# tumberger/gnark-fork

Hardware: AMD Instinct MI355X
Metric: Groth16 prove time + MSM G1 throughput (Mscalar-mul/s) BN254 2^24 R1CS, 1/2/4/8 GPU (higher is better)
Workload: dtype u32 limbs (BN254 Fp/Fr Montgomery, integer)

## Files before the change

### gnark-fork_amd/csrc/groth16.hip

```cpp
#include "common.h"
#include "curve.cuh"
#include "stage.h"
#include <chrono>
#include <future>
#include <memory>
#include <mutex>
#include <thread>
#include <vector>
#include <cstdlib>
#include <cstring>

struct gg_domain;
struct gg_msm_base;

namespace gg {
struct MsmSort;
struct MsmScratch;
struct MsmWork;
void compute_h_device(gg_domain* d, Fr* A, Fr* B, Fr* C, Fr* H, hipStream_t st);
void msm_device(gg_msm_base* b, const Fr* scalars_dev, void* out_jac, hipStream_t st);
size_t msm_scalars_needed(gg_msm_base* b);
gg_msm_base* msm_base_create_internal(int group, const void* host_points, size_t n,
                                      const uint32_t* sidx, int window_bits, bool keep_inf, int groups);
int choose_groups_multi(const double* bytes, const int* W, int k, double extra);
bool msm_same_shape(const gg_msm_base* a, const gg_msm_base* b);
MsmSort* msm_own_sort(gg_msm_base* b);
void msm_prepare_dev(gg_msm_base* b, MsmSort* s, const Fr* scalars_dev, hipStream_t st, int slog = 0,
                     uint32_t sres = 0);
void msm_finish_dev(gg_msm_base* b, MsmSort* s, void* out_jac, hipStream_t st, MsmScratch* scr = nullptr);
MsmWork* msm_work_new();
void msm_work_delete(MsmWork* w);
MsmSort* msm_work_sort(MsmWork* w);
void msm_prepare_derived_dev(gg_msm_base* a, MsmSort* sa, gg_msm_base* b, MsmSort* sb, const uint32_t* bmap,
                             hipStream_t st);
bool msm_derivable(const gg_msm_base* a, const gg_msm_base* b);
void msm_build_bmap(const gg_msm_base* a, const gg_msm_base* b, DevBuf& bmap);
MsmScratch* msm_work_scratch(MsmWork* w);
int msm_base_window(const gg_msm_base* b);
int choose_c(size_t n, size_t point_bytes, int total_bits);
void hshard_run(gg_hshard* hs, const Fr* a, const Fr* b, const Fr* c, size_t len, bool compact, Fr* send,
                Fr* recv, gg_exchange_fn xchg, void* ctx, hipStream_t st);
size_t hshard_m(const gg_hshard* hs, int* rank, int* world, int* log_n);
Fr* hshard_h(gg_hshard* hs);
int hshard_curve(const gg_hshard* hs);
}

struct DistH {
    gg_hshard* hs;
    gg_exchange_fn xchg;
    void* ctx;
    gg::Fr *send, *recv;
};

using namespace gg;

struct CurveBn254 {
    using FrT = Fr;
    using G1F = Fp;
    using G2F = Fp2;
    static constexpr int curve = GG_CURVE_BN254, g1 = GG_G1, g2 = GG_G2, total_bits = 255;
};
struct CurveBls12381 {
    using FrT = FrBls;
    using G1F = FpBls;
    using G2F = Fp2Bls;
    static constexpr int curve = GG_CURVE_BLS12_381, g1 = GG_BLS12_381_G1, g2 = GG_BLS12_381_G2, total_bits = 256;
};
struct PointSizes {
    size_t g1a, g2a, g1j, g2j;
};
static PointSizes point_sizes(int curve) {
    if (curve == GG_CURVE_BN254) return {64, 128, 96, 192};
// ... 5 lines not shown
    bool share_AK = false, share_B = false;
    bool derive_B = false;
    DevBuf bmap;
    int groups = 1;
    WireBases() = default;
    WireBases(const WireBases&) = delete;
    WireBases& operator=(const WireBases&) = delete;
    ~WireBases() {
        for (gg_msm_base_t b : {A, B, K, B2})
            if (b) gg_msm_base_release(b);
    }
};

struct WorkSet {
    MsmWork *A = nullptr, *B = nullptr, *K = nullptr, *B2 = nullptr;
    WorkSet() {
        A = msm_work_new();
        B = msm_work_new();
        K = msm_work_new();
        B2 = msm_work_new();
    }
    WorkSet(const WorkSet&) = delete;
    WorkSet& operator=(const WorkSet&) = delete;
    ~WorkSet() {
        for (MsmWork* w : {A, B, K, B2})
            if (w) msm_work_delete(w);
    }
};

struct gg_groth16_pk {
    int curve = GG_CURVE_BN254;
    int log_n = 0;
    size_t n = 0;
    gg_domain_t dom = nullptr;
    std::shared_ptr<WireBases> wb;
    gg_msm_base_t A = nullptr, B = nullptr, K = nullptr, Z = nullptr, B2 = nullptr;
    int slog = 0;
    uint32_t spart = 0;
    std::unique_ptr<WorkSet> work;
    uint8_t alpha[96], beta[96], delta[96], beta2[192], delta2[192];
    size_t n_wires = 0, nb_public = 0;
    size_t wire_lo = 0, wire_hi = 0, z_lo = 0, nZ = 0;
    bool share_AK = false, share_B = false;
    DevBuf wires, sa, sb, sc;
    hipStream_t s0 = nullptr, s1 = nullptr, s2 = nullptr, s3 = nullptr, s4 = nullptr;
    TaskQueue tq[5];
    hipStream_t* const* active() {
        act[0] = &s0, act[1] = &s1, act[2] = &s2, act[3] = &s3, act[4] = &s4;
        return act;
    }
    hipStream_t* act[5] = {};
    hipStream_t hprio = nullptr;
    std::unique_ptr<Stager> stager;
    int device = 0;
    std::mutex mu;
    ~gg_groth16_pk() {
        stager.reset();
        work.reset();
        wb.reset();
        if (Z) gg_msm_base_release(Z);
        if (dom) gg_domain_release(dom);
        task_streams_release(tq, 5, device);
        if (hprio) (void)hipStreamDestroy(hprio);
    }
};

static thread_local double g_timings[9];
static thread_local double g_ext[3];

static void ck(int rc) {
    if (rc != GG_OK) throw Error(rc, gg_last_error());
}

static std::shared_ptr<WireBases> wire_bases_build(int curve, int log_n, const void* g1_A, size_t nA,
                                                   const void* g1_B, size_t nB, const void* g1_K, size_t nK,
                                                   const void* g2_B, const uint8_t* inf_A, const uint8_t* inf_B,
                                                   size_t n_wires, size_t nb_public, const uint32_t* k_wire_index,
                                                   size_t lo, size_t hi, size_t nZ) {
    GG_CHECK(inf_A && inf_B, GG_ERR_INVALID_ARG, "null infinity masks");
    GG_CHECK(nb_public <= n_wires, GG_ERR_INVALID_ARG, "nb_public > n_wires");
    GG_CHECK(lo <= hi && hi <= n_wires, GG_ERR_INVALID_ARG, "bad wire shard range");
    GG_CHECK(curve == GG_CURVE_BN254 || curve == GG_CURVE_BLS12_381, GG_ERR_INVALID_ARG, "bad curve");
    const PointSizes ps = point_sizes(curve);
    const int g1 = curve == GG_CURVE_BN254 ? GG_G1 : GG_BLS12_381_G1;
    const int g2 = curve == GG_CURVE_BN254 ? GG_G2 : GG_BLS12_381_G2;
    const int tbits = curve == GG_CURVE_BN254 ? 255 : 256;
    std::vector<uint32_t> ia, ib, ik;
    for (size_t i = lo; i < hi; i++) {
        if (!inf_A[i]) ia.push_back((uint32_t)(i - lo));
        if (!inf_B[i]) ib.push_back((uint32_t)(i - lo));
    }
    GG_CHECK(ia.size() == nA, GG_ERR_INVALID_ARG, "len(pk.G1.A) != n_wires - NbInfinityA (shard)");
    GG_CHECK(ib.size() == nB, GG_ERR_INVALID_ARG, "len(pk.G1.B) != n_wires - NbInfinityB (shard)");
    ik.resize(nK);
    const size_t k0 = std::max(lo, nb_public);
    for (size_t i = 0; i < nK; i++) {
        size_t w = k_wire_index ? (size_t)k_wire_index[i] : k0 + i;
        GG_CHECK(w >= lo && w < hi, GG_ERR_INVALID_ARG, "K wire index outside the shard");
        ik[i] = (uint32_t)(w - lo);
    }
    GG_CHECK(nA == 0 || g1_A, GG_ERR_INVALID_ARG, "null g1_A");
    GG_CHECK(nB == 0 || (g1_B && g2_B), GG_ERR_INVALID_ARG, "null g1_B / g2_B");
    GG_CHECK(nK == 0 || g1_K, GG_ERR_INVALID_ARG, "null g1_K");
    const size_t nw = hi - lo;
    const int cAK = choose_c(std::max<size_t>(nw, 1), ps.g1a, tbits);
    int cB = choose_c(std::max<size_t>(nB, 1), 128, tbits);
    const bool try_derive = getenv("GG_G16_B_DERIVE") && atoi(getenv("GG_G16_B_DERIVE")) != 0;
    if (try_derive && cAK >= cB && cAK - cB <= 2 && nB) cB = cAK;
    if (const char* e = getenv("GG_G16_B_WINDOW")) cB = std::max(4, std::min(24, atoi(e)));
// ... 39 lines not shown
                      const void* omega_mont, const void* coset_gen_mont, const void* g1_Z, size_t z_lo, size_t nZ,
                      const void* alpha1, const void* beta1, const void* delta1, const void* beta2,
                      const void* delta2, size_t n_wires, size_t nb_public, size_t lo, size_t hi, int slog,
                      uint32_t spart) {
    GG_CHECK(omega_mont && coset_gen_mont && alpha1 && beta1 && delta1 && beta2 && delta2,
             GG_ERR_INVALID_ARG, "null argument");
    GG_CHECK(log_n >= 0 && log_n <= 28, GG_ERR_INVALID_ARG, "log_n out of range");
    const PointSizes ps = point_sizes(curve);
    const int g1 = curve == GG_CURVE_BN254 ? GG_G1 : GG_BLS12_381_G1;
    const int tbits = curve == GG_CURVE_BN254 ? 255 : 256;
    pk->curve = curve;
    pk->log_n = log_n;
    pk->n = (size_t)1 << log_n;
    pk->n_wires = n_wires;
    pk->nb_public = nb_public;
    pk->wire_lo = lo;
    pk->wire_hi = hi;
    pk->z_lo = z_lo;
    pk->nZ = nZ;
    const size_t nz_full = pk->n > 1 ? pk->n - 1 : 0;
    GG_CHECK(z_lo + nZ <= nz_full, GG_ERR_INVALID_ARG,
             "Z shard beyond domain cardinality - 1 (setup.go:266)");
    GG_CHECK(nZ == 0 || g1_Z, GG_ERR_INVALID_ARG, "null g1_Z");
    GG_HIP(hipGetDevice(&pk->device));
    memcpy(pk->alpha, alpha1, ps.g1a);
    memcpy(pk->beta, beta1, ps.g1a);
    memcpy(pk->delta, delta1, ps.g1a);
    memcpy(pk->beta2, beta2, ps.g2a);
    memcpy(pk->delta2, delta2, ps.g2a);
    ck(gg_domain_create_ex(curve, log_n, omega_mont, coset_gen_mont, &pk->dom));
    pk->wb = std::move(wb);
    pk->A = pk->wb->A;
    pk->B = pk->wb->B;
    pk->K = pk->wb->K;
    pk->B2 = pk->wb->B2;
    pk->share_AK = pk->wb->share_AK;
    pk->share_B = pk->wb->share_B;
    if (slog) {
        int cmin = 64;
        for (gg_msm_base_t b : {pk->A, pk->B})
            if (msm_scalars_needed(b)) cmin = std::min(cmin, msm_base_window(b));
        GG_CHECK(slog <= cmin - 2, GG_ERR_INVALID_ARG, "bucket stripe too fine for the tables' windows");
        GG_CHECK(spart < (1u << slog), GG_ERR_INVALID_ARG, "stripe part out of range");
        pk->slog = slog;
        pk->spart = spart;
        pk->work.reset(new WorkSet());
    }
    const int cZ = choose_c(std::max<size_t>(nZ, 1), ps.g1a, tbits);
    pk->Z = msm_base_create_internal(g1, g1_Z, nZ, nullptr, cZ, false, pk->wb->groups);
    int cur = 0;
    GG_HIP(hipGetDevice(&cur));
    task_streams_init(pk->active(), pk->tq, 5, cur, true);
    h_priority_ab(pk);
}

static void pk_build(gg_groth16_pk* pk, int curve, int log_n, const void* omega_mont, const void* coset_gen_mont,
                     const void* g1_A, size_t nA, const void* g1_B, size_t nB, const void* g1_Z,
                     size_t z_lo, size_t nZ, const void* g1_K, size_t nK, const void* alpha1,
                     const void* beta1, const void* delta1, const void* g2_B, const void* beta2,
                     const void* delta2, const uint8_t* inf_A, const uint8_t* inf_B, size_t n_wires,
                     size_t nb_public, const uint32_t* k_wire_index, size_t lo, size_t hi) {
    GG_CHECK(log_n >= 0 && log_n <= 28, GG_ERR_INVALID_ARG, "log_n out of range");
    auto wb = wire_bases_build(curve, log_n, g1_A, nA, g1_B, nB, g1_K, nK, g2_B, inf_A, inf_B, n_wires, nb_public,
                               k_wire_index, lo, hi, nZ);
    pk_finish(pk, std::move(wb), curve, log_n, omega_mont, coset_gen_mont, g1_Z, z_lo, nZ, alpha1, beta1, delta1,
              beta2, delta2, n_wires, nb_public, lo, hi, 0, 0);
}

namespace gg {
std::shared_ptr<WireBases> g16_wire_bases(int curve, int log_n, const void* g1_A, size_t nA, const void* g1_B,
                                          size_t nB, const void* g1_K, size_t nK, const void* g2_B,
                                          const uint8_t* inf_A, const uint8_t* inf_B, size_t n_wires,
                                          size_t nb_public, const uint32_t* k_wire_index, size_t nZ) {
    return wire_bases_build(curve, log_n, g1_A, nA, g1_B, nB, g1_K, nK, g2_B, inf_A, inf_B, n_wires, nb_public,
                            k_wire_index, 0, n_wires, nZ);
}
gg_groth16_pk* g16_stripe_shard(std::shared_ptr<WireBases> wb, int curve, int log_n, const void* omega_mont,
                                const void* coset_gen_mont, const void* g1_Z, size_t z_lo, size_t nZ,
                                const void* alpha1, const void* beta1, const void* delta1, const void* beta2,
                                const void* delta2, size_t n_wires, size_t nb_public, int slog, uint32_t spart) {
    std::unique_ptr<gg_groth16_pk> pk(new gg_groth16_pk());
    pk_finish(pk.get(), std::move(wb), curve, log_n, omega_mont, coset_gen_mont, g1_Z, z_lo, nZ, alpha1, beta1,
              delta1, beta2, delta2, n_wires, nb_public, 0, n_wires, slog, spart);
    return pk.release();
}
int g16_wire_window(int curve, size_t n_wires, size_t nB) {
    const PointSizes ps = point_sizes(curve);
    const int tbits = curve == GG_CURVE_BN254 ? 255 : 256;
    int c = 64;
    if (n_wires) c = std::min(c, choose_c(n_wires, ps.g1a, tbits));
    if (nB) c = std::min(c, choose_c(nB, 128, tbits));
    return c;
}
void g16_restream(gg_groth16_pk* pk, bool dedicated) {
    std::lock_guard<std::mutex> lk(pk->mu);
    task_streams_switch(pk->active(), pk->tq, 5, pk->device, dedicated);
    h_priority_ab(pk);
}
}

extern "C" int gg_groth16_pk_create_ex(int curve, int log_n, const void* omega_mont, const void* coset_gen_mont,
                                       const void* g1_A, size_t nA, const void* g1_B, size_t nB,
                                       const void* g1_Z, size_t nZ, const void* g1_K, size_t nK,
                                       const void* alpha1, const void* beta1, const void* delta1,
                                       const void* g2_B, const void* beta2, const void* delta2,
                                       const uint8_t* inf_A, const uint8_t* inf_B, size_t n_wires,
// ... 120 lines not shown
        .count();
}

template <class T>
static T from_bytes(const void* p) {
    T x;
    memcpy(&x, p, sizeof(T));
    return x;
}

struct G16Partials {
    alignas(16) uint8_t a[144], b1[144], k[144], z[144];
    alignas(16) uint8_t b2[288];
};
static void set_g1_inf(int curve, void* p) {
    if (curve == GG_CURVE_BN254) {
        G1Jac j = G1Jac::inf();
        memcpy(p, &j, sizeof(j));
    } else {
        Jac<FpBls> j = Jac<FpBls>::inf();
        memcpy(p, &j, sizeof(j));
    }
}
static void partials_put(int curve, const G16Partials& p, void* out) {
    const PointSizes ps = point_sizes(curve);
    uint8_t* o = (uint8_t*)out;
    memcpy(o, p.a, ps.g1j);
    memcpy(o + ps.g1j, p.b1, ps.g1j);
    memcpy(o + 2 * ps.g1j, p.k, ps.g1j);
    memcpy(o + 3 * ps.g1j, p.z, ps.g1j);
    memcpy(o + 4 * ps.g1j, p.b2, ps.g2j);
}
static void partials_get(int curve, const void* in, G16Partials& p) {
    const PointSizes ps = point_sizes(curve);
    const uint8_t* q = (const uint8_t*)in;
    memcpy(p.a, q, ps.g1j);
    memcpy(p.b1, q + ps.g1j, ps.g1j);
    memcpy(p.k, q + 2 * ps.g1j, ps.g1j);
    memcpy(p.z, q + 3 * ps.g1j, ps.g1j);
    memcpy(p.b2, q + 4 * ps.g1j, ps.g2j);
}

struct Joiner {
    std::vector<gg::Task<void>>& v;
    ~Joiner() {
        for (auto& t : v)
            if (t.valid()) t.wait();
    }
};

static void prove_device(gg_groth16_pk* pk, const void* wires, const void* sol_a,
                         const void* sol_b, const void* sol_c, size_t n_cons,
                         bool inputs_on_device, void* h_dev_out, G16Partials& out,
                         const DistH* dh = nullptr) {
    double t0 = now_ms();
    const size_t n = pk->n;
    const size_t nbytes = n * 32;
    const size_t nw_shard = pk->wire_hi - pk->wire_lo;
    const Fr* wdev = (const Fr*)wires;
    if (!inputs_on_device) {
        if (!pk->stager) pk->stager.reset(new Stager(pk->device));
        pk->wires.reserve(std::max<size_t>(nw_shard, 1) * 32);
        pk->stager->upload(pk->wires.p, (const uint8_t*)wires + pk->wire_lo * 32, nw_shard * 32);
        const hipStream_t cons[4] = {pk->s0, pk->s2, pk->s3, pk->s4};
        pk->stager->ready(cons, 4);
        wdev = pk->wires.as<Fr>();
    } else {
        wdev += pk->wire_lo;
    }
    double t_up = now_ms();

    set_g1_inf(pk->curve, out.z);
    double t_h = 0, t_z = 0, t_a = 0, t_b = 0, t_k = 0, t_upabc = 0;
    std::mutex emu;
    std::string werr;
    int wcode = GG_OK;
    const int dev = pk->device;
    auto guarded = [&](auto fn) {
        return [&, fn]() {
            try {
                GG_HIP(hipSetDevice(dev));
                fn();
            } catch (const Error& e) {
                std::lock_guard<std::mutex> g(emu);
                if (wcode == GG_OK) { werr = e.what(); wcode = e.code; }
            } catch (const std::exception& e) {
                std::lock_guard<std::mutex> g(emu);
                if (wcode == GG_OK) { werr = e.what(); wcode = GG_ERR_INTERNAL; }
            }
        };
    };
    const bool serial = getenv("GG_G16_SERIAL") && atoi(getenv("GG_G16_SERIAL"));
    std::vector<gg::Task<void>> workers;
    Joiner joiner{workers};
    auto spawn = [&](auto fn) {
        if (serial) fn();
        else workers.push_back(gg::run_task(fn));
    };
    auto inputs_abc = [&](Fr*& A, Fr*& B, Fr*& C, size_t& len) {
        const void* src[3] = {sol_a, sol_b, sol_c};
        Fr* dst[3] = {pk->sa.as<Fr>(), pk->sb.as<Fr>(), pk->sc.as<Fr>()};
        len = n_cons;
        const double a = now_ms();
        if (inputs_on_device) {
            for (int i = 0; i < 3; i++) {
                if (dh) { dst[i] = (Fr*)src[i]; continue; }
                if (n_cons) GG_HIP(hipMemcpyAsync(dst[i], src[i], n_cons * 32, hipMemcpyDeviceToDevice, pk->s1));
                if (n_cons < n) GG_HIP(hipMemsetAsync((char*)dst[i] + n_cons * 32, 0, nbytes - n_cons * 32, pk->s1));
            }
        } else if (dh) {
            int rank = 0, world = 1, lg = 0;
            hshard_m(dh->hs, &rank, &world, &lg);
            len = n_cons > (size_t)rank ? (n_cons - (size_t)rank + world - 1) / world : 0;
            for (int i = 0; i < 3; i++)
                pk->stager->upload_strided(dst[i], src[i], 32, (size_t)rank, (size_t)world, len);
            pk->stager->ready(&pk->s1, 1);
        } else {
            for (int i = 0; i < 3; i++) {
                if (n_cons < n) GG_HIP(hipMemsetAsync((char*)dst[i] + n_cons * 32, 0, nbytes - n_cons * 32, pk->s1));
                pk->stager->upload(dst[i], src[i], n_cons * 32);
            }
            pk->stager->ready(&pk->s1, 1);
        }
        t_upabc = now_ms() - a;
        A = dst[0];
        B = dst[1];
        C = dst[2];
    };
    pk->sa.reserve(nbytes);
    pk->sb.reserve(nbytes);
    pk->sc.reserve(nbytes);
    if (dh) spawn(guarded([&] {
        Fr *A, *B, *C;
        size_t len;
        double a = now_ms();
        inputs_abc(A, B, C, len);
        const bool compact = !inputs_on_device;
        hshard_run(dh->hs, A, B, C, len, compact, dh->send, dh->recv, dh->xchg, dh->ctx, pk->s1);
        GG_WAIT_STREAM(pk->s1);
        double b = now_ms();
        t_h = b - a;
        msm_device(pk->Z, hshard_h(dh->hs), out.z, pk->s1);
        t_z = now_ms() - b;
    }));
    else spawn(guarded([&] {
        Fr *A, *B, *C;
        size_t len;
        double a = now_ms();
        inputs_abc(A, B, C, len);
        compute_h_device(pk->dom, A, B, C, A, pk->s1);
        GG_WAIT_STREAM(pk->s1);
        double b = now_ms();
        t_h = b - a;
        if (h_dev_out) GG_HIP(hipMemcpyAsync(h_dev_out, A, nbytes, hipMemcpyDeviceToDevice, pk->s1));
        if (n > 1) msm_device(pk->Z, A + pk->z_lo, out.z, pk->s1);
        t_z = now_ms() - b;
    }));
    MsmSort *sAK = nullptr, *sB = nullptr, *sK = nullptr, *sB2 = nullptr;
    MsmScratch *xA = nullptr, *xB = nullptr, *xK = nullptr, *xB2 = nullptr;
    WorkSet* ws = pk->work.get();
    guarded([&] {
        sAK = ws ? msm_work_sort(ws->A) : msm_own_sort(pk->A);
        sB = ws ? msm_work_sort(ws->B) : msm_own_sort(pk->B);
        sK = pk->share_AK ? sAK : (ws ? msm_work_sort(ws->K) : msm_own_sort(pk->K));
        sB2 = pk->share_B ? sB : (ws ? msm_work_sort(ws->B2) : msm_own_sort(pk->B2));
        if (ws) {
            xA = msm_work_scratch(ws->A);
            xB = msm_work_scratch(ws->B);
            xK = msm_work_scratch(ws->K);
            xB2 = msm_work_scratch(ws->B2);
        }
        msm_prepare_dev(pk->A, sAK, wdev, pk->s2, pk->slog, pk->spart);
        if (pk->wb->derive_B)
            msm_prepare_derived_dev(pk->A, sAK, pk->B, sB, pk->wb->bmap.as<uint32_t>(), pk->s3);
        else
            msm_prepare_dev(pk->B, sB, wdev, pk->s3, pk->slog, pk->spart);
        if (!pk->share_AK) msm_prepare_dev(pk->K, sK, wdev, pk->s4, pk->slog, pk->spart);
        if (!pk->share_B) msm_prepare_dev(pk->B2, sB2, wdev, pk->s0, pk->slog, pk->spart);
    })();
    double t2 = now_ms(), te = t2;
    if (wcode == GG_OK) {
        spawn(guarded([&] { double a = now_ms(); msm_finish_dev(pk->A, sAK, out.a, pk->s2, xA); t_a = now_ms() - a; }));
        spawn(guarded([&] { double a = now_ms(); msm_finish_dev(pk->B, sB, out.b1, pk->s3, xB); t_b = now_ms() - a; }));
        spawn(guarded([&] { double a = now_ms(); msm_finish_dev(pk->K, sK, out.k, pk->s4, xK); t_k = now_ms() - a; }));
        t2 = now_ms();
        guarded([&] { msm_finish_dev(pk->B2, sB2, out.b2, pk->s0, xB2); })();
        te = now_ms();
    }
    for (auto& w : workers) w.wait();
    if (wcode != GG_OK) throw Error(wcode, werr);
    g_timings[0] = t_up - t0;
    g_timings[1] = t_h;
    g_timings[2] = t_a;
    g_timings[3] = t_b;
    g_timings[4] = t_k;
    g_timings[5] = t_z;
    g_timings[6] = te - t2;
    g_ext[0] = t_upabc;
}

template <class Cv>
struct G16Fixed {
    typename Cv::FrT rc, sc;
    Jac<typename Cv::G1F> rd, sd, krd;
    Jac<typename Cv::G2F> sd2;
};

template <class Cv>
static gg::Task<G16Fixed<Cv>> fixed_terms_async(const void* delta_aff, const void* delta2_aff, const void* r_mont,
                                                   const void* s_mont) {
    using G1 = typename Cv::G1F;
    using G2 = typename Cv::G2F;
    using FrT = typename Cv::FrT;
    const Affine<G1> delta = from_bytes<Affine<G1>>(delta_aff);
    const Affine<G2> delta2 = from_bytes<Affine<G2>>(delta2_aff);
    const FrT r = from_bytes<FrT>(r_mont), s = from_bytes<FrT>(s_mont);
    return gg::run_task([delta, delta2, r, s] {
        G16Fixed<Cv> f;
        FrT kr = -(r * s);
        f.rc = from_mont(r);
        f.sc = from_mont(s);
        FrT krc = from_mont(kr);
        Jac<G1> dl = Jac<G1>::from_affine(delta);
        auto f_rd = gg::run_task([&] { return jac_mul(dl, f.rc.v); });
        auto f_sd = gg::run_task([&] { return jac_mul(dl, f.sc.v); });
        auto f_sd2 = gg::run_task([&] { return jac_mul(Jac<G2>::from_affine(delta2), f.sc.v); });
        f.krd = jac_mul(dl, krc.v);
        f.rd = f_rd.get();
        f.sd = f_sd.get();
        f.sd2 = f_sd2.get();
        return f;
    });
}

template <class Cv>
static void g16_combine(const G16Partials& p, const G16Fixed<Cv>& f, const void* alpha_aff, const void* beta_aff,
                        const void* beta2_aff, void* ar_aff, void* bs_aff, void* krs_aff) {
    using G1 = typename Cv::G1F;
    using G2 = typename Cv::G2F;
    const Affine<G1> alpha = from_bytes<Affine<G1>>(alpha_aff), beta = from_bytes<Affine<G1>>(beta_aff);
    const Affine<G2> beta2 = from_bytes<Affine<G2>>(beta2_aff);
    const Jac<G1> pa = from_bytes<Jac<G1>>(p.a), pb1 = from_bytes<Jac<G1>>(p.b1), pk = from_bytes<Jac<G1>>(p.k),
                  pz = from_bytes<Jac<G1>>(p.z);
    const Jac<G2> pb2 = from_bytes<Jac<G2>>(p.b2);
    Jac<G1> ar = jac_add(jac_add_affine(pa, alpha), f.rd);
    Jac<G1> bs1 = jac_add(jac_add_affine(pb1, beta), f.sd);
    auto f_sar = gg::run_task([&] { return jac_mul(ar, f.sc.v); });
    Jac<G1> rbs = jac_mul(bs1, f.rc.v);
    Jac<G1> krs = jac_add(jac_add(pk, f.krd), pz);
    krs = jac_add(krs, f_sar.get());
    krs = jac_add(krs, rbs);
    Jac<G2> bs = jac_add_affine(jac_add(pb2, f.sd2), beta2);
    const Affine<G1> o_ar = jac_to_affine(ar), o_krs = jac_to_affine(krs);
    const Affine<G2> o_bs = jac_to_affine(bs);
    memcpy(ar_aff, &o_ar, sizeof(o_ar));
    memcpy(krs_aff, &o_krs, sizeof(o_krs));
    memcpy(bs_aff, &o_bs, sizeof(o_bs));
}

template <class Cv>
static void prove_whole(gg_groth16_pk* pk, const void* wires, const void* sol_a, const void* sol_b,
                        const void* sol_c, size_t n_cons, bool on_dev, const void* r_mont, const void* s_mont,
                        void* ar_aff, void* bs_aff, void* krs_aff, void* h_dev_out) {
    double t0 = now_ms();
    auto fixed = fixed_terms_async<Cv>(pk->delta, pk->delta2, r_mont, s_mont);
    G16Partials p;
    prove_device(pk, wires, sol_a, sol_b, sol_c, n_cons, on_dev, h_dev_out, p);
    double tep = now_ms();
    g16_combine<Cv>(p, fixed.get(), pk->alpha, pk->beta, pk->beta2, ar_aff, bs_aff, krs_aff);
    double tend = now_ms();
    g_timings[7] = tend - tep;
    g_timings[8] = tend - t0;
}

static void check_prove_args(gg_groth16_pk_t pk, const void* wires, size_t n_wires, const void* a,
                             const void* b, const void* c, size_t n_cons) {
    GG_CHECK(pk && wires && a && b && c, GG_ERR_INVALID_ARG, "null argument");
    GG_CHECK(n_wires == pk->n_wires, GG_ERR_INVALID_ARG, "len(wires) != pk wires");
    GG_CHECK(n_cons <= pk->n, GG_ERR_INVALID_ARG, "nbConstraints > domain cardinality");
}

extern "C" int gg_groth16_prove(gg_groth16_pk_t pk, const void* wires, size_t n_wires,
                                const void* sol_a, const void* sol_b, const void* sol_c,
                                size_t n_cons, int inputs_on_device, const void* r_mont,
                                const void* s_mont, void* ar_aff, void* bs_aff, void* krs_aff,
                                void* h_dev_out) {
    GG_CAPI_BEGIN
    check_prove_args(pk, wires, n_wires, sol_a, sol_b, sol_c, n_cons);
    GG_CHECK(r_mont && s_mont && ar_aff && bs_aff && krs_aff, GG_ERR_INVALID_ARG, "null argument");
    GG_CHECK(pk->wire_lo == 0 && pk->wire_hi == pk->n_wires && pk->z_lo == 0 && pk->slog == 0 &&
                 pk->nZ == (pk->n > 1 ? pk->n - 1 : 0),
             GG_ERR_INVALID_ARG, "gg_groth16_prove needs the whole key; a shard proves with "
                                 "gg_groth16_prove_partial + gg_groth16_finalize");
    g_ext[1] = now_ms();
    std::lock_guard<std::mutex> lk(pk->mu);
    g_ext[0] = 0;
    if (pk->curve == GG_CURVE_BN254)
        prove_whole<CurveBn254>(pk, wires, sol_a, sol_b, sol_c, n_cons, inputs_on_device != 0, r_mont, s_mont,
                                ar_aff, bs_aff, krs_aff, h_dev_out);
    else
        prove_whole<CurveBls12381>(pk, wires, sol_a, sol_b, sol_c, n_cons, inputs_on_device != 0, r_mont, s_mont,
                                   ar_aff, bs_aff, krs_aff, h_dev_out);
    g_ext[2] = now_ms();
    if (kAccumProbe) {
        set_last_error("traffic-probe build (GG_ACCUM_PROBE): the MSM sums are wrong, the proof is NOT valid");
        return GG_REHEARSAL;
    }
    GG_CAPI_END
}

extern "C" int gg_groth16_prove_partial(gg_groth16_pk_t pk, const void* wires, size_t n_wires,
                                        const void* sol_a, const void* sol_b, const void* sol_c,
                                        size_t n_cons, int inputs_on_device, void* partials,
                                        void* h_dev_out) {
    GG_CAPI_BEGIN
    check_prove_args(pk, wires, n_wires, sol_a, sol_b, sol_c, n_cons);
    GG_CHECK(partials, GG_ERR_INVALID_ARG, "null argument");
    std::lock_guard<std::mutex> lk(pk->mu);
    g_ext[0] = 0;
    double t0 = now_ms();
// ... 117 lines not shown
```

### gnark-fork_amd/csrc/ntt.hip

```cpp
#include "common.h"
#include "field.cuh"
#include "prof.h"
#include <vector>
#include <mutex>
#include <memory>
#include <algorithm>
#include <cstring>
#include <type_traits>

namespace gg {

enum ScaleKind {
    SK_G_NAT = 0,
    SK_G_BR = 1,
    SK_GINV_NAT_N = 2,
    SK_GINV_BR_N = 3,
    SK_NINV = 4,
    SK_H_FWD = 5,
    SK_H_INV = 6,
    SK_DEN_N = 7,
    SK_COUNT = 8
};

template <class F>
struct ScaleSpec {
    const F* hi;
    const F* lo;
    int shift;
    int bitrev;
};

template <class F>
struct PassParams {
    const F* in;
    F* out;
    const F* tw;
    int log_n;
    int b_lo;
    int k;
    int tl;
    int dit;
    int has_pre;
    ScaleSpec<F> pre;
    int has_post;
    ScaleSpec<F> post;
    int epi_mul_sub;
    int epi_mul;
    int epi_sub;
    const F* ea;
    const F* eb;
    int canon_out;
};

template <class F>
struct NttLazy {
    static constexpr bool on = false;
};
template <>
struct NttLazy<Fr> {
    static constexpr bool on = true;
};
template <class C>
GG_HD constexpr uint32_t twop_limb(int i) {
    uint64_t c = 0;
    uint32_t v = 0;
    for (int j = 0; j <= i; j++) {
        const uint64_t t = (uint64_t)C::P[j] * 2 + c;
        v = (uint32_t)t;
        c = t >> 32;
    }
    return v;
}
template <class C>
__device__ __forceinline__ Fe<C> red2p(const Fe<C>& x) {
    Fe<C> s, r;
    uint32_t br = 0;
#pragma unroll
    for (int i = 0; i < 8; i++) s.v[i] = __builtin_subc(x.v[i], twop_limb<C>(i), br, &br);
#pragma unroll
    for (int i = 0; i < 8; i++) r.v[i] = br ? x.v[i] : s.v[i];
    return r;
}
template <class C>
__device__ __forceinline__ Fe<C> add2p(const Fe<C>& a, const Fe<C>& b) {
    Fe<C> r;
    uint32_t c = 0;
#pragma unroll
    for (int i = 0; i < 8; i++) r.v[i] = __builtin_addc(a.v[i], b.v[i], c, &c);
    return red2p(r);
}
template <class C>
__device__ __forceinline__ Fe<C> subnr2p(const Fe<C>& a, const Fe<C>& b) {
    Fe<C> r;
    uint32_t br = 0, c = 0;
#pragma unroll
    for (int i = 0; i < 8; i++) r.v[i] = __builtin_subc(a.v[i], b.v[i], br, &br);
#pragma unroll
    for (int i = 0; i < 8; i++) r.v[i] = __builtin_addc(r.v[i], twop_limb<C>(i), c, &c);
    return r;
}
template <class C>
__device__ __forceinline__ Fe<C> sub2p(const Fe<C>& a, const Fe<C>& b) {
    Fe<C> r, s;
    uint32_t br = 0, c = 0;
// ... 1 lines not shown
    for (int i = 0; i < 8; i++) r.v[i] = __builtin_subc(a.v[i], b.v[i], br, &br);
#pragma unroll
    for (int i = 0; i < 8; i++) s.v[i] = __builtin_addc(r.v[i], twop_limb<C>(i), c, &c);
#pragma unroll
    for (int i = 0; i < 8; i++) r.v[i] = br ? s.v[i] : r.v[i];
    return r;
}
template <class C>
__device__ __forceinline__ Fe<C> canon(const Fe<C>& x) {
    Fe<C> s, r;
    uint32_t br = 0;
#pragma unroll
    for (int i = 0; i < 8; i++) s.v[i] = __builtin_subc(x.v[i], C::P[i], br, &br);
#pragma unroll
    for (int i = 0; i < 8; i++) r.v[i] = br ? x.v[i] : s.v[i];
    return r;
}

__device__ __forceinline__ uint32_t brev_bits(uint32_t i, int L) {
    return L ? (__brev(i) >> (32 - L)) : 0u;
}

template <class F>
__device__ __forceinline__ F apply_scale(const ScaleSpec<F>& s, uint32_t g, int L, const F& x) {
    uint32_t e = s.bitrev ? brev_bits(g, L) : g;
    F f = ld_fr(s.hi + (e >> s.shift));
    if (s.lo) f = f * ld_fr(s.lo + (e & ((1u << s.shift) - 1)));
    return x * f;
}

__device__ __forceinline__ int lidx(int e) { return e + (e >> 5); }

template <class F, int NB, bool DIT>
__device__ __forceinline__ void ntt_round(const PassParams<F>& P, uint32_t* lds, int TP, int T, int qlo,
                                          bool first, bool last, uint32_t base_hi, uint32_t lo0) {
    constexpr int R = 1 << NB;
    const int tl = P.tl;
    const uint32_t tl_mask = (1u << tl) - 1;
    const int pos = qlo + tl;
    const uint32_t lowmask = (1u << pos) - 1;
    const int groups = T >> NB;
    for (int gi = threadIdx.x; gi < groups; gi += blockDim.x) {
        uint32_t e[R], g[R];
        F x[R];
        const uint32_t low = (uint32_t)gi & lowmask, high = ((uint32_t)gi >> pos) << (pos + NB);
#pragma unroll
        for (int m = 0; m < R; m++) {
            e[m] = high | ((uint32_t)m << pos) | low;
            g[m] = base_hi | ((e[m] >> tl) << P.b_lo) | (lo0 + (e[m] & tl_mask));
        }
        if (first) {
#pragma unroll
            for (int m = 0; m < R; m++) {
                x[m] = ld_fr(P.in + g[m]);
                if (P.has_pre) x[m] = apply_scale(P.pre, g[m], P.log_n, x[m]);
            }
        } else {
#pragma unroll
            for (int m = 0; m < R; m++) {
#pragma unroll
                for (int l = 0; l < 8; l++) x[m].v[l] = lds[l * TP + lidx((int)e[m])];
            }
        }
#pragma unroll
        for (int s2 = 0; s2 < NB; s2++) {
            const int r = DIT ? s2 : (NB - 1 - s2);
            const int b = P.b_lo + qlo + r;
            const uint32_t bmask = (1u << b) - 1;
            const F* twb = P.tw + bmask;
#pragma unroll
            for (int m = 0; m < R; m++) {
                if (m & (1 << r)) continue;
                const int m2 = m | (1 << r);
                const uint32_t i = g[m] & bmask;
                if constexpr (NttLazy<F>::on) {
                    if (DIT) {
                        F t = i ? mul_nored(x[m2], ld_fr(twb + i)) : x[m2];
                        x[m2] = sub2p(x[m], t);
                        x[m] = add2p(x[m], t);
                    } else {
                        F d = subnr2p(x[m], x[m2]);
                        x[m] = add2p(x[m], x[m2]);
                        x[m2] = i ? mul_nored(d, ld_fr(twb + i)) : red2p(d);
                    }
                    continue;
                }
                if (DIT) {
                    F t = i ? x[m2] * ld_fr(twb + i) : x[m2];
                    x[m2] = x[m] - t;
                    x[m] = x[m] + t;
                } else {
                    F d = x[m] - x[m2];
                    x[m] = x[m] + x[m2];
                    x[m2] = i ? d * ld_fr(twb + i) : d;
                }
            }
        }
        if (last) {
#pragma unroll
            for (int m = 0; m < R; m++) {
                F y = x[m];
                if (NttLazy<F>::on && P.canon_out && !P.has_post) y = canon(y);
                if (P.has_post) y = apply_scale(P.post, g[m], P.log_n, y);
                if (P.epi_mul_sub) y = ld_fr(P.ea + g[m]) * ld_fr(P.eb + g[m]) - y;
                if (P.epi_mul) y = ld_fr(P.ea + g[m]) * y;
                if (P.epi_sub) y = y - ld_fr(P.ea + g[m]);
                st_fr(P.out + g[m], y);
            }
        } else {
#pragma unroll
            for (int m = 0; m < R; m++) {
#pragma unroll
                for (int l = 0; l < 8; l++) lds[l * TP + lidx((int)e[m])] = x[m].v[l];
            }
        }
    }
}

template <int MAXNB>
constexpr int kNttThreads = MAXNB == 3 ? 256 : (MAXNB == 2 ? 512 : 1024);
template <int MAXNB>
constexpr int kNttWaves = MAXNB == 3 ? 1 : (MAXNB == 2 ? 4 : 8);
template <class F, bool DIT, int MAXNB>
__global__ void __launch_bounds__(kNttThreads<MAXNB>, kNttWaves<MAXNB>) k_ntt_pass(PassParams<F> P) {
    extern __shared__ __attribute__((aligned(16))) uint32_t lds[];
    const int k = P.k, tl = P.tl;
    const int T = 1 << (k + tl);
    const int TP = T + (T >> 5);
    const int nlo_log = P.b_lo - tl;
    const uint32_t tile = blockIdx.x;
    const uint32_t lob = tile & ((1u << nlo_log) - 1);
    const uint32_t hi = tile >> nlo_log;
    const uint32_t base_hi = hi << (P.b_lo + k);
    const uint32_t lo0 = lob << tl;
    if (k == 0) {
        for (int e = threadIdx.x; e < T; e += blockDim.x) {
            uint32_t g = base_hi | (lo0 + (uint32_t)e);
            F x = ld_fr(P.in + g);
            if (P.has_pre) x = apply_scale(P.pre, g, P.log_n, x);
            if (P.has_post) x = apply_scale(P.post, g, P.log_n, x);
            if (P.epi_mul_sub) x = ld_fr(P.ea + g) * ld_fr(P.eb + g) - x;
            if (P.epi_mul) x = ld_fr(P.ea + g) * x;
            if (P.epi_sub) x = x - ld_fr(P.ea + g);
            st_fr(P.out + g, x);
        }
        return;
    }
    int done = 0;
    bool first = true;
    while (done < k) {
        const int nb = min(MAXNB, k - done);
        const int qlo = DIT ? done : (k - done - nb);
        const bool last = (done + nb == k);
        if (!first) __syncthreads();
        if constexpr (MAXNB >= 3) {
            if (nb == 3) {
                ntt_round<F, 3, DIT>(P, lds, TP, T, qlo, first, last, base_hi, lo0);
                first = false;
                done += nb;
                continue;
            }
        }
        if constexpr (MAXNB >= 2) {
            if (nb == 2) {
                ntt_round<F, 2, DIT>(P, lds, TP, T, qlo, first, last, base_hi, lo0);
                first = false;
                done += nb;
                continue;
            }
        }
        ntt_round<F, 1, DIT>(P, lds, TP, T, qlo, first, last, base_hi, lo0);
        first = false;
        done += nb;
    }
}

template <class F>
__global__ void k_stage_twiddles(F* out, size_t count, int L, const F* hi, const F* lo, int S) {
    size_t t = (size_t)blockIdx.x * blockDim.x + threadIdx.x;
    if (t >= count) return;
    uint32_t v = (uint32_t)t + 1;
    int b = 31 - __clz((int)v);
    uint32_t i = v - (1u << b);
    uint32_t ex = i << (L - 1 - b);
    F x = ld_fr(hi + (ex >> S)) * ld_fr(lo + (ex & ((1u << S) - 1)));
    st_fr(out + t, x);
}


struct Pass {
    int b_lo, k, tl;
// ... 29 lines not shown
    int log_n = 0;
    size_t n = 1;
    F omega, omega_inv, g, g_inv, n_inv, den;
    DevBuf tw, twinv;
    int S = 0;
    DevBuf scale_hi[SK_COUNT], scale_lo[SK_COUNT];
    ScaleSpec<F> spec[SK_COUNT];
};
}

struct gg_domain {
    int curve = GG_CURVE_BN254;
    int log_n = 0;
    size_t n = 1;
    std::unique_ptr<DomainT<FrCfg>> bn;
    std::unique_ptr<DomainT<FrBlsCfg>> bls;
    DevBuf scratch;
    std::mutex mu;
};

namespace gg {

template <class F>
static void build_pow_tables(int L, int S, const F& x, const F& c, std::vector<F>& hi,
                             std::vector<F>& lo) {
    size_t nlo = (size_t)1 << S, nhi = (size_t)1 << (L - S);
    lo.resize(nlo);
    hi.resize(nhi);
    F acc = F::one();
    for (size_t i = 0; i < nlo; i++) { lo[i] = acc; acc = acc * x; }
    F step = acc;
    acc = c;
    for (size_t i = 0; i < nhi; i++) { hi[i] = acc; acc = acc * step; }
}

template <class F>
static void upload(DevBuf& b, const std::vector<F>& v) {
    b.alloc(v.size() * sizeof(F));
    GG_HIP(hipMemcpy(b.p, v.data(), v.size() * sizeof(F), hipMemcpyHostToDevice));
}

static int ntt_radix() {
    const char* e = getenv("GG_NTT_RADIX");
    const int r = e ? atoi(e) : 4;
    return (r == 2 || r == 8) ? r : 4;
}

static hipStream_t pick_stream(void* s) { return s ? (hipStream_t)s : hipStreamPerThread; }

enum { EPI_MUL_SUB = 0, EPI_MUL = 1, EPI_SUB = 2 };
template <class C>
void run_transform(DomainT<C>* d, const Fe<C>* in, Fe<C>* out, bool dit, bool inverse_tw, int pre_kind,
                   int post_kind, const Fe<C>* ea, const Fe<C>* eb, hipStream_t st, int epi = EPI_MUL_SUB,
                   const std::vector<Pass>* only = nullptr) {
    using F = Fe<C>;
    const int L = d->log_n;
    auto passes = only ? *only : plan_passes(L, dit);
    const F* src = in;
    for (size_t pi = 0; pi < passes.size(); pi++) {
        const Pass& ps = passes[pi];
        PassParams<F> P{};
        P.in = src;
        P.out = out;
        P.tw = (const F*)(inverse_tw ? d->twinv.p : d->tw.p);
        P.log_n = L;
        P.b_lo = ps.b_lo;
        P.k = ps.k;
        P.tl = ps.tl;
        P.dit = dit ? 1 : 0;
        if (pi == 0 && pre_kind >= 0) { P.has_pre = 1; P.pre = d->spec[pre_kind]; }
        bool last = (pi + 1 == passes.size());
        if (last && post_kind >= 0) { P.has_post = 1; P.post = d->spec[post_kind]; }
        if (last && ea) {
            P.epi_mul_sub = epi == EPI_MUL_SUB;
            P.epi_mul = epi == EPI_MUL;
            P.epi_sub = epi == EPI_SUB;
            P.ea = ea;
            P.eb = eb;
        }
        P.canon_out = last ? 1 : 0;
        int T = 1 << (ps.k + ps.tl);
        unsigned tiles = (unsigned)(d->n / (size_t)T);
        size_t lds = (ps.k > 3) ? (size_t)(T + (T >> 5)) * 32 : 0;
        ProfScope prof("ntt_pass", st, (double)d->n);
        static const int radix = ntt_radix();
        if (radix == 4) {
            lds = (ps.k > 2) ? (size_t)(T + (T >> 5)) * 32 : 0;
            if (dit) hipLaunchKernelGGL((k_ntt_pass<F, true, 2>), dim3(tiles), dim3(512), lds, st, P);
            else hipLaunchKernelGGL((k_ntt_pass<F, false, 2>), dim3(tiles), dim3(512), lds, st, P);
        } else if (radix == 2) {
            lds = (ps.k > 1) ? (size_t)(T + (T >> 5)) * 32 : 0;
            if (dit) hipLaunchKernelGGL((k_ntt_pass<F, true, 1>), dim3(tiles), dim3(1024), lds, st, P);
            else hipLaunchKernelGGL((k_ntt_pass<F, false, 1>), dim3(tiles), dim3(1024), lds, st, P);
        } else {
            if (dit) hipLaunchKernelGGL((k_ntt_pass<F, true, 3>), dim3(tiles), dim3(256), lds, st, P);
            else hipLaunchKernelGGL((k_ntt_pass<F, false, 3>), dim3(tiles), dim3(256), lds, st, P);
        }
        GG_HIP(hipGetLastError());
        prof.stop(st);
        src = out;
    }
}

}

namespace gg {
template <class C>
static DomainT<C>* domain_build(int log_n, const void* omega_mont, const void* coset_gen_mont) {
    using F = Fe<C>;
    std::unique_ptr<DomainT<C>> d(new DomainT<C>());
    d->log_n = log_n;
    d->n = (size_t)1 << log_n;
    memcpy(d->omega.v, omega_mont, 32);
    memcpy(d->g.v, coset_gen_mont, 32);
    F x = d->omega;
    for (int i = 0; i < log_n; i++) {
// ... 67 lines not shown
    run_transform(d, a, a, dit, inverse != 0, pre, post, (const Fe<C>*)nullptr, (const Fe<C>*)nullptr, st);
}
}

extern "C" int gg_domain_create_ex(int curve, int log_n, const void* omega_mont,
                                   const void* coset_gen_mont, gg_domain_t* out) {
    GG_CAPI_BEGIN
    GG_CHECK(out && omega_mont && coset_gen_mont, GG_ERR_INVALID_ARG, "null argument");
    GG_CHECK(curve == GG_CURVE_BN254 || curve == GG_CURVE_BLS12_381, GG_ERR_INVALID_ARG, "bad curve");
    GG_CHECK(log_n >= 0 && log_n <= (curve == GG_CURVE_BN254 ? 28 : 30), GG_ERR_INVALID_ARG,
             "log_n out of range");
    std::unique_ptr<gg_domain> d(new gg_domain());
    d->curve = curve;
    d->log_n = log_n;
    d->n = (size_t)1 << log_n;
    if (curve == GG_CURVE_BN254) d->bn.reset(domain_build<FrCfg>(log_n, omega_mont, coset_gen_mont));
    else d->bls.reset(domain_build<FrBlsCfg>(log_n, omega_mont, coset_gen_mont));
    *out = d.release();
    GG_CAPI_END
}

extern "C" int gg_domain_create(int log_n, const void* omega_mont, const void* coset_gen_mont,
                                gg_domain_t* out) {
    return gg_domain_create_ex(GG_CURVE_BN254, log_n, omega_mont, coset_gen_mont, out);
}

extern "C" int gg_domain_release(gg_domain_t d) {
    GG_CAPI_BEGIN
    delete d;
    GG_CAPI_END
}

extern "C" int gg_domain_log_n(gg_domain_t d, int* log_n) {
    GG_CAPI_BEGIN
    GG_CHECK(d && log_n, GG_ERR_INVALID_ARG, "null argument");
    *log_n = d->log_n;
    GG_CAPI_END
}

extern "C" int gg_ntt(gg_domain_t d, void* data_dev, int inverse, int decimation, int coset,
                      void* hip_stream) {
    GG_CAPI_BEGIN
    GG_CHECK(d && data_dev, GG_ERR_INVALID_ARG, "null argument");
    GG_CHECK(decimation == GG_DIF || decimation == GG_DIT, GG_ERR_INVALID_ARG, "bad decimation");
    hipStream_t st = pick_stream(hip_stream);
    bool dit = decimation == GG_DIT;
    if (d->curve == GG_CURVE_BN254) ntt_apply(d->bn.get(), data_dev, inverse, dit, coset, st);
    else ntt_apply(d->bls.get(), data_dev, inverse, dit, coset, st);
    GG_CAPI_END
}

namespace gg {
template <class C>
static void compute_h_t(DomainT<C>* d, Fe<C>* A, Fe<C>* B, Fe<C>* Cv, Fe<C>* H, hipStream_t st) {
    const Fe<C>* nul = nullptr;
    run_transform(d, A, A, false, true, -1, SK_H_FWD, nul, nul, st);
    run_transform(d, A, A, true, false, -1, -1, nul, nul, st);
    run_transform(d, B, B, false, true, -1, SK_H_FWD, nul, nul, st);
    run_transform(d, B, B, true, false, -1, -1, (const Fe<C>*)A, nul, st, EPI_MUL);
    run_transform(d, Cv, Cv, false, true, -1, SK_DEN_N, nul, nul, st);
    GG_CHECK(H != Cv, GG_ERR_INTERNAL, "computeH: h must not alias c");
    run_transform(d, B, H, false, true, -1, SK_H_INV, (const Fe<C>*)Cv, nul, st, EPI_SUB);
}
void compute_h_device(gg_domain* dom, Fr* A, Fr* B, Fr* C, Fr* H, hipStream_t st) {
    if (dom->curve == GG_CURVE_BN254) compute_h_t(dom->bn.get(), A, B, C, H, st);
    else compute_h_t(dom->bls.get(), (FrBls*)A, (FrBls*)B, (FrBls*)C, (FrBls*)H, st);
}
}

extern "C" int gg_groth16_compute_h(gg_domain_t d, const void* a, const void* b, const void* c,
                                    size_t len, int inputs_on_device, void* h_dev,
                                    void* hip_stream) {
    GG_CAPI_BEGIN
    GG_CHECK(d && a && b && c && h_dev, GG_ERR_INVALID_ARG, "null argument");
    GG_CHECK(len <= d->n, GG_ERR_INVALID_ARG, "len > domain cardinality");
    std::lock_guard<std::mutex> lk(d->mu);
    hipStream_t st = pick_stream(hip_stream);
    size_t nb = d->n * 32;
    d->scratch.reserve(3 * nb);
    char* base = (char*)d->scratch.p;
    Fr* A = (Fr*)base;
    Fr* B = (Fr*)(base + nb);
    Fr* C = (Fr*)(base + 2 * nb);
    hipMemcpyKind kind = inputs_on_device ? hipMemcpyDeviceToDevice : hipMemcpyHostToDevice;
    const void* src[3] = {a, b, c};
    Fr* dst[3] = {A, B, C};
    for (int i = 0; i < 3; i++) {
        if (len) GG_HIP(hipMemcpyAsync(dst[i], src[i], len * 32, kind, st));
        if (len < d->n) GG_HIP(hipMemsetAsync((char*)dst[i] + len * 32, 0, nb - len * 32, st));
    }
    compute_h_device(d, A, B, C, (Fr*)h_dev, st);
    GG_WAIT_STREAM(st);
    GG_CAPI_END
}

namespace gg {
size_t domain_size(gg_domain* d, int* curve) {
    if (curve) *curve = d->curve;
    return d->n;
}
void any_ntt_inplace(gg_domain* d, void* data, int inverse, int dit, int coset, hipStream_t st) {
    if (d->curve == GG_CURVE_BN254) ntt_apply(d->bn.get(), data, inverse, dit != 0, coset, st);
    else ntt_apply(d->bls.get(), data, inverse, dit != 0, coset, st);
}
void ntt_inverse_dit_noscale(gg_domain* d, void* data, hipStream_t st) {
    if (d->curve == GG_CURVE_BN254)
        run_transform(d->bn.get(), (const Fr*)data, (Fr*)data, true, true, -1, -1, (const Fr*)nullptr,
                      (const Fr*)nullptr, st);
    else
        run_transform(d->bls.get(), (const FrBls*)data, (FrBls*)data, true, true, -1, -1, (const FrBls*)nullptr,
                      (const FrBls*)nullptr, st);
}
void ntt_tail_inverse_coset(gg_domain* d, void* data, int u, hipStream_t st) {
    const int L = d->log_n;
    GG_CHECK(u >= 1 && u <= 4 && L >= 12, GG_ERR_INTERNAL, "tail transform: 1..4 stages of a >= 2^12 domain");
    const std::vector<Pass> tail = {{L - u, u, 11 - u}};
    if (d->curve == GG_CURVE_BN254)
        run_transform(d->bn.get(), (const Fr*)data, (Fr*)data, true, true, -1, SK_GINV_NAT_N, (const Fr*)nullptr,
                      (const Fr*)nullptr, st, EPI_MUL_SUB, &tail);
    else
        run_transform(d->bls.get(), (const FrBls*)data, (FrBls*)data, true, true, -1, SK_GINV_NAT_N,
                      (const FrBls*)nullptr, (const FrBls*)nullptr, st, EPI_MUL_SUB, &tail);
}
template <class C>
static void xn_minus_one_inv_t(const DomainT<C>* d, size_t n_small, void* out) {
    using F = Fe<C>;
    const size_t rho = d->n / n_small;
    std::vector<F> res(rho);
    res[0] = pow_u64(d->g, n_small);
    const F t = pow_u64(d->omega, n_small);
    for (size_t i = 1; i < rho; i++) res[i] = res[i - 1] * t;
    for (size_t i = 0; i < rho; i++) {
        res[i] = res[i] - F::one();
        GG_CHECK(!res[i].is_zero(), GG_ERR_INVALID_ARG, "x^n - 1 vanishes on the big coset");
        res[i] = inverse(res[i]);
    }
    memcpy(out, res.data(), rho * sizeof(F));
}
void xn_minus_one_inv(gg_domain* big, size_t n_small, void* out) {
    if (big->curve == GG_CURVE_BN254) xn_minus_one_inv_t(big->bn.get(), n_small, out);
    else xn_minus_one_inv_t(big->bls.get(), n_small, out);
}
}

// ... 486 lines not shown
```

Measured before the change: 159.3 million.

## Read device inputs directly in first NTT pass and optionally enqueue H ahead

For device-resident inputs, the device-to-device copy and zero-padding of A, B, C before computing H are removed. The first NTT pass now reads from the source buffers out of place and substitutes zero past the input length. H timing now uses events rather than host waits. A new GG_G16_ORDER option can enqueue H on the calling thread before the MSMs start and gate the MSM finish steps on an H-done event. That option defaults to 'task', so only the copy removal is on by default; it adds a bounds check per load in the first pass.

Measured after the change: 160.5 million (median of 6 runs). Within noise of the previous version (+0.8%).

```diff
diff --git a/gnark-fork_amd/csrc/groth16.hip b/gnark-fork_amd/csrc/groth16.hip
--- a/gnark-fork_amd/csrc/groth16.hip
+++ b/gnark-fork_amd/csrc/groth16.hip
@@ -18,6 +18,8 @@
 struct MsmScratch;
 struct MsmWork;
 void compute_h_device(gg_domain* d, Fr* A, Fr* B, Fr* C, Fr* H, hipStream_t st);
+void compute_h_device(gg_domain* d, const Fr* srcA, const Fr* srcB, const Fr* srcC, size_t len, Fr* A, Fr* B, Fr* C,
+                      Fr* H, hipStream_t st);
 void msm_device(gg_msm_base* b, const Fr* scalars_dev, void* out_jac, hipStream_t st);
 size_t msm_scalars_needed(gg_msm_base* b);
 gg_msm_base* msm_base_create_internal(int group, const void* host_points, size_t n,
@@ -129,9 +131,16 @@
     hipStream_t* act[5] = {};
     hipStream_t hprio = nullptr;
     std::unique_ptr<Stager> stager;
+    hipEvent_t ev_h[3] = {};
+    void events() {
+        for (auto& e : ev_h)
+            if (!e) GG_HIP(hipEventCreate(&e));
+    }
     int device = 0;
     std::mutex mu;
     ~gg_groth16_pk() {
+        for (auto e : ev_h)
+            if (e) (void)hipEventDestroy(e);
         stager.reset();
         work.reset();
         wb.reset();
@@ -277,6 +286,7 @@
     GG_HIP(hipGetDevice(&cur));
     task_streams_init(pk->active(), pk->tq, 5, cur, true);
     h_priority_ab(pk);
+    pk->events();
 }
 
 static void pk_build(gg_groth16_pk* pk, int curve, int log_n, const void* omega_mont, const void* coset_gen_mont,
@@ -503,7 +513,7 @@
 static void prove_device(gg_groth16_pk* pk, const void* wires, const void* sol_a,
                          const void* sol_b, const void* sol_c, size_t n_cons,
                          bool inputs_on_device, void* h_dev_out, G16Partials& out,
-                         const DistH* dh = nullptr) {
+                         const DistH* dh = nullptr, bool whole = false) {
     double t0 = now_ms();
     const size_t n = pk->n;
     const size_t nbytes = n * 32;
@@ -542,6 +552,15 @@
         };
     };
     const bool serial = getenv("GG_G16_SERIAL") && atoi(getenv("GG_G16_SERIAL"));
+    enum { ORD_TASK, ORD_FIRST, ORD_GATE3, ORD_GATE };
+    int order = ORD_TASK;
+    if (const char* e = getenv("GG_G16_ORDER")) {
+        const std::string v(e);
+        GG_CHECK(v == "task" || v == "first" || v == "gate3" || v == "gate" || v.empty(), GG_ERR_INVALID_ARG,
+                 "GG_G16_ORDER: task, first, gate3 or gate");
+        order = v == "gate" ? ORD_GATE : (v == "gate3" ? ORD_GATE3 : (v == "first" ? ORD_FIRST : ORD_TASK));
+    }
+    const bool ahead = whole && inputs_on_device && !dh && !serial && order != ORD_TASK;
     std::vector<gg::Task<void>> workers;
     Joiner joiner{workers};
     auto spawn = [&](auto fn) {
@@ -554,11 +573,8 @@
         len = n_cons;
         const double a = now_ms();
         if (inputs_on_device) {
-            for (int i = 0; i < 3; i++) {
-                if (dh) { dst[i] = (Fr*)src[i]; continue; }
-                if (n_cons) GG_HIP(hipMemcpyAsync(dst[i], src[i], n_cons * 32, hipMemcpyDeviceToDevice, pk->s1));
-                if (n_cons < n) GG_HIP(hipMemsetAsync((char*)dst[i] + n_cons * 32, 0, nbytes - n_cons * 32, pk->s1));
-            }
+            for (int i = 0; i < 3; i++)
+                if (dh) dst[i] = (Fr*)src[i];
         } else if (dh) {
             int rank = 0, world = 1, lg = 0;
             hshard_m(dh->hs, &rank, &world, &lg);
@@ -581,6 +597,29 @@
     pk->sa.reserve(nbytes);
     pk->sb.reserve(nbytes);
     pk->sc.reserve(nbytes);
+    auto h_enqueue = [&] {
+        Fr *A, *B, *C;
+        size_t len;
+        GG_HIP(hipEventRecord(pk->ev_h[0], pk->s1));
+        inputs_abc(A, B, C, len);
+        if (inputs_on_device)
+            compute_h_device(pk->dom, (const Fr*)sol_a, (const Fr*)sol_b, (const Fr*)sol_c, n_cons, A, B, C, A, pk->s1);
+        else
+            compute_h_device(pk->dom, A, B, C, A, pk->s1);
+        GG_HIP(hipEventRecord(pk->ev_h[1], pk->s1));
+    };
+    auto z_run = [&] {
+        Fr* A = pk->sa.as<Fr>();
+        if (h_dev_out) GG_HIP(hipMemcpyAsync(h_dev_out, A, nbytes, hipMemcpyDeviceToDevice, pk->s1));
+        if (n > 1) msm_device(pk->Z, A + pk->z_lo, out.z, pk->s1);
+        GG_HIP(hipEventRecord(pk->ev_h[2], pk->s1));
+        GG_WAIT_EVENT(pk->ev_h[2]);
+        float ms_h = 0, ms_z = 0;
+        GG_HIP(hipEventElapsedTime(&ms_h, pk->ev_h[0], pk->ev_h[1]));
+        GG_HIP(hipEventElapsedTime(&ms_z, pk->ev_h[1], pk->ev_h[2]));
+        t_h = ms_h;
+        t_z = ms_z;
+    };
     if (dh) spawn(guarded([&] {
         Fr *A, *B, *C;
         size_t len;
@@ -594,19 +633,12 @@
         msm_device(pk->Z, hshard_h(dh->hs), out.z, pk->s1);
         t_z = now_ms() - b;
     }));
-    else spawn(guarded([&] {
-        Fr *A, *B, *C;
-        size_t len;
-        double a = now_ms();
-        inputs_abc(A, B, C, len);
-        compute_h_device(pk->dom, A, B, C, A, pk->s1);
-        GG_WAIT_STREAM(pk->s1);
-        double b = now_ms();
-        t_h = b - a;
-        if (h_dev_out) GG_HIP(hipMemcpyAsync(h_dev_out, A, nbytes, hipMemcpyDeviceToDevice, pk->s1));
-        if (n > 1) msm_device(pk->Z, A + pk->z_lo, out.z, pk->s1);
-        t_z = now_ms() - b;
-    }));
+    else if (ahead) {
+        guarded(h_enqueue)();
+        if (wcode == GG_OK) spawn(guarded(z_run));
+    } else {
+        spawn(guarded([&] { h_enqueue(); z_run(); }));
+    }
     MsmSort *sAK = nullptr, *sB = nullptr, *sK = nullptr, *sB2 = nullptr;
     MsmScratch *xA = nullptr, *xB = nullptr, *xK = nullptr, *xB2 = nullptr;
     WorkSet* ws = pk->work.get();
@@ -630,12 +662,17 @@
         if (!pk->share_B) msm_prepare_dev(pk->B2, sB2, wdev, pk->s0, pk->slog, pk->spart);
     })();
     double t2 = now_ms(), te = t2;
+    const bool gate1 = ahead && (order == ORD_GATE || order == ORD_GATE3), gate2 = ahead && order == ORD_GATE;
+    auto finish = [&](gg_msm_base_t b, MsmSort* s, void* o, hipStream_t st, MsmScratch* x, bool gate) {
+        if (gate) GG_HIP(hipStreamWaitEvent(st, pk->ev_h[1], 0));
+        msm_finish_dev(b, s, o, st, x);
+    };
     if (wcode == GG_OK) {
-        spawn(guarded([&] { double a = now_ms(); msm_finish_dev(pk->A, sAK, out.a, pk->s2, xA); t_a = now_ms() - a; }));
-        spawn(guarded([&] { double a = now_ms(); msm_finish_dev(pk->B, sB, out.b1, pk->s3, xB); t_b = now_ms() - a; }));
-        spawn(guarded([&] { double a = now_ms(); msm_finish_dev(pk->K, sK, out.k, pk->s4, xK); t_k = now_ms() - a; }));
+        spawn(guarded([&] { double a = now_ms(); finish(pk->A, sAK, out.a, pk->s2, xA, gate1); t_a = now_ms() - a; }));
+        spawn(guarded([&] { double a = now_ms(); finish(pk->B, sB, out.b1, pk->s3, xB, gate1); t_b = now_ms() - a; }));
+        spawn(guarded([&] { double a = now_ms(); finish(pk->K, sK, out.k, pk->s4, xK, gate1); t_k = now_ms() - a; }));
         t2 = now_ms();
-        guarded([&] { msm_finish_dev(pk->B2, sB2, out.b2, pk->s0, xB2); })();
+        guarded([&] { finish(pk->B2, sB2, out.b2, pk->s0, xB2, gate2); })();
         te = now_ms();
     }
     for (auto& w : workers) w.wait();
@@ -716,7 +753,7 @@
     double t0 = now_ms();
     auto fixed = fixed_terms_async<Cv>(pk->delta, pk->delta2, r_mont, s_mont);
     G16Partials p;
-    prove_device(pk, wires, sol_a, sol_b, sol_c, n_cons, on_dev, h_dev_out, p);
+    prove_device(pk, wires, sol_a, sol_b, sol_c, n_cons, on_dev, h_dev_out, p, nullptr, true);
     double tep = now_ms();
     g16_combine<Cv>(p, fixed.get(), pk->alpha, pk->beta, pk->beta2, ar_aff, bs_aff, krs_aff);
     double tend = now_ms();
diff --git a/gnark-fork_amd/csrc/ntt.hip b/gnark-fork_amd/csrc/ntt.hip
--- a/gnark-fork_amd/csrc/ntt.hip
+++ b/gnark-fork_amd/csrc/ntt.hip
@@ -50,6 +50,7 @@
     const F* ea;
     const F* eb;
     int canon_out;
+    uint32_t in_len;
 };
 
 template <class F>
@@ -157,7 +158,7 @@
         if (first) {
 #pragma unroll
             for (int m = 0; m < R; m++) {
-                x[m] = ld_fr(P.in + g[m]);
+                x[m] = g[m] < P.in_len ? ld_fr(P.in + g[m]) : F::zero();
                 if (P.has_pre) x[m] = apply_scale(P.pre, g[m], P.log_n, x[m]);
             }
         } else {
@@ -241,7 +242,7 @@
     if (k == 0) {
         for (int e = threadIdx.x; e < T; e += blockDim.x) {
             uint32_t g = base_hi | (lo0 + (uint32_t)e);
-            F x = ld_fr(P.in + g);
+            F x = g < P.in_len ? ld_fr(P.in + g) : F::zero();
             if (P.has_pre) x = apply_scale(P.pre, g, P.log_n, x);
             if (P.has_post) x = apply_scale(P.post, g, P.log_n, x);
             if (P.epi_mul_sub) x = ld_fr(P.ea + g) * ld_fr(P.eb + g) - x;
@@ -377,16 +378,18 @@
 template <class C>
 void run_transform(DomainT<C>* d, const Fe<C>* in, Fe<C>* out, bool dit, bool inverse_tw, int pre_kind,
                    int post_kind, const Fe<C>* ea, const Fe<C>* eb, hipStream_t st, int epi = EPI_MUL_SUB,
-                   const std::vector<Pass>* only = nullptr) {
+                   const std::vector<Pass>* only = nullptr, size_t in_len = SIZE_MAX) {
     using F = Fe<C>;
     const int L = d->log_n;
     auto passes = only ? *only : plan_passes(L, dit);
     const F* src = in;
+    GG_CHECK(in_len >= d->n || in != out, GG_ERR_INTERNAL, "a short input is transformed out of place");
     for (size_t pi = 0; pi < passes.size(); pi++) {
         const Pass& ps = passes[pi];
         PassParams<F> P{};
         P.in = src;
         P.out = out;
+        P.in_len = (uint32_t)(pi == 0 ? std::min(in_len, d->n) : d->n);
         P.tw = (const F*)(inverse_tw ? d->twinv.p : d->tw.p);
         P.log_n = L;
         P.b_lo = ps.b_lo;
@@ -560,19 +563,28 @@
 
 namespace gg {
 template <class C>
-static void compute_h_t(DomainT<C>* d, Fe<C>* A, Fe<C>* B, Fe<C>* Cv, Fe<C>* H, hipStream_t st) {
+static void compute_h_t(DomainT<C>* d, const Fe<C>* srcA, const Fe<C>* srcB, const Fe<C>* srcC, size_t len,
+                        Fe<C>* A, Fe<C>* B, Fe<C>* Cv, Fe<C>* H, hipStream_t st) {
     const Fe<C>* nul = nullptr;
-    run_transform(d, A, A, false, true, -1, SK_H_FWD, nul, nul, st);
+    const std::vector<Pass>* all = nullptr;
+    GG_CHECK(len <= d->n, GG_ERR_INTERNAL, "computeH: input longer than the domain");
+    run_transform(d, srcA, A, false, true, -1, SK_H_FWD, nul, nul, st, EPI_MUL_SUB, all, len);
     run_transform(d, A, A, true, false, -1, -1, nul, nul, st);
-    run_transform(d, B, B, false, true, -1, SK_H_FWD, nul, nul, st);
+    run_transform(d, srcB, B, false, true, -1, SK_H_FWD, nul, nul, st, EPI_MUL_SUB, all, len);
     run_transform(d, B, B, true, false, -1, -1, (const Fe<C>*)A, nul, st, EPI_MUL);
-    run_transform(d, Cv, Cv, false, true, -1, SK_DEN_N, nul, nul, st);
+    run_transform(d, srcC, Cv, false, true, -1, SK_DEN_N, nul, nul, st, EPI_MUL_SUB, all, len);
     GG_CHECK(H != Cv, GG_ERR_INTERNAL, "computeH: h must not alias c");
     run_transform(d, B, H, false, true, -1, SK_H_INV, (const Fe<C>*)Cv, nul, st, EPI_SUB);
 }
+void compute_h_device(gg_domain* dom, const Fr* srcA, const Fr* srcB, const Fr* srcC, size_t len, Fr* A, Fr* B,
+                      Fr* C, Fr* H, hipStream_t st) {
+    if (dom->curve == GG_CURVE_BN254) compute_h_t(dom->bn.get(), srcA, srcB, srcC, len, A, B, C, H, st);
+    else
+        compute_h_t(dom->bls.get(), (const FrBls*)srcA, (const FrBls*)srcB, (const FrBls*)srcC, len, (FrBls*)A,
+                    (FrBls*)B, (FrBls*)C, (FrBls*)H, st);
+}
 void compute_h_device(gg_domain* dom, Fr* A, Fr* B, Fr* C, Fr* H, hipStream_t st) {
-    if (dom->curve == GG_CURVE_BN254) compute_h_t(dom->bn.get(), A, B, C, H, st);
-    else compute_h_t(dom->bls.get(), (FrBls*)A, (FrBls*)B, (FrBls*)C, (FrBls*)H, st);
+    compute_h_device(dom, A, B, C, dom->n, A, B, C, H, st);
 }
 }
 
@@ -590,14 +602,17 @@
     Fr* A = (Fr*)base;
     Fr* B = (Fr*)(base + nb);
     Fr* C = (Fr*)(base + 2 * nb);
-    hipMemcpyKind kind = inputs_on_device ? hipMemcpyDeviceToDevice : hipMemcpyHostToDevice;
-    const void* src[3] = {a, b, c};
-    Fr* dst[3] = {A, B, C};
-    for (int i = 0; i < 3; i++) {
-        if (len) GG_HIP(hipMemcpyAsync(dst[i], src[i], len * 32, kind, st));
-        if (len < d->n) GG_HIP(hipMemsetAsync((char*)dst[i] + len * 32, 0, nb - len * 32, st));
-    }
-    compute_h_device(d, A, B, C, (Fr*)h_dev, st);
+    if (inputs_on_device) {
+        compute_h_device(d, (const Fr*)a, (const Fr*)b, (const Fr*)c, len, A, B, C, (Fr*)h_dev, st);
+    } else {
+        const void* src[3] = {a, b, c};
+        Fr* dst[3] = {A, B, C};
+        for (int i = 0; i < 3; i++) {
+            if (len) GG_HIP(hipMemcpyAsync(dst[i], src[i], len * 32, hipMemcpyHostToDevice, st));
+            if (len < d->n) GG_HIP(hipMemsetAsync((char*)dst[i] + len * 32, 0, nb - len * 32, st));
+        }
+        compute_h_device(d, A, B, C, (Fr*)h_dev, st);
+    }
     GG_WAIT_STREAM(st);
     GG_CAPI_END
 }
```
